# JuliaLinearAlgebra/AlgebraicMultigrid.jl

Measured on AMD Instinct MI355X. Metric: V-cycle unknowns/sec + fine-level SpMV GB/s (% HBM peak), 3-D Poisson 256^3, higher is better.
Workload: dtype f64

## Files before the change

### algebraicmultigrid.jl_amd/_libs.py

```python
import ctypes as C
import os

_HERE = os.path.dirname(os.path.abspath(__file__))
SETUP_SO = os.path.join(_HERE, "libamgsetup.so")
HIP_SO = os.path.join(_HERE, "libamghip.so")
HIP_F32_SO = os.path.join(_HERE, "libamghip_f32.so")

i32p = C.POINTER(C.c_int32)
f64p = C.POINTER(C.c_double)
i64 = C.c_int64
vp = C.c_void_p


class AMGError(RuntimeError):
    pass


class amgs_options(C.Structure):
    _fields_ = [("theta", C.c_double), ("max_levels", C.c_int32), ("max_coarse", C.c_int32),
                ("hermitian", C.c_int32), ("sa_omega", C.c_double), ("sa_improve_iters", C.c_int32),
                ("sa_B_is_vector", C.c_int32)]


class amgh_smoother_t(C.Structure):
# ... 144 lines not shown
    L.amgh_stream.restype = vp
    L.amgh_stream.argtypes = [vp]
    L.amgh_timer_begin.argtypes = [vp]
    L.amgh_timer_end.argtypes = [vp, C.POINTER(C.c_double)]
    L.amgh_bench_op.argtypes = [vp, C.c_int, C.c_int, C.c_int, C.c_int, C.POINTER(C.c_double)]
    L.amgh_debug_chain_timing.argtypes = [C.c_int, vp]
    L.amgh_debug_merged_sweep_host.argtypes = [i64, i64, vp, vp, vp, C.c_int, C.c_int, C.c_double, vp, vp]
    L.amgh_debug_bw_poll_giveups.argtypes = [vp, C.c_int]
    L.amgh_debug_bw_mode.argtypes = [vp, C.c_int]
    L.amgh_debug_bw_dict.argtypes = [vp, C.c_int]
    L.amgh_debug_bw_late.argtypes = [vp, C.c_int]
    L.amgh_debug_coded_ops.argtypes = [vp, C.c_int]
    L.amgh_debug_bw_sweep_host.argtypes = [i64, vp, vp, vp, C.c_int, C.c_int, C.c_double, vp, vp, vp]
    L.amgh_debug_bw_dict_sweep_host.argtypes = [i64, vp, vp, vp, C.c_int, C.c_int, vp, vp, vp]
    L.amgh_debug_set_tunable.argtypes = [C.c_char_p, C.c_int]
    L.amgh_debug_get_tunable.argtypes = [C.c_char_p, C.POINTER(C.c_int)]
    L.amgh_profile_enable.argtypes = [vp, C.c_int]
    L.amgh_profile_read.argtypes = [vp, vp, C.c_int]
    L.amgh_set_use_graph.argtypes = [vp, C.c_int]


def _bind_dist(L):
    i64p = C.POINTER(i64)
    L.amgh_dist_rccl_available.argtypes = []
    L.amgh_dist_unique_id.argtypes = [vp]
    L.amgh_dist_create_rccl.argtypes = [C.POINTER(vp), C.c_int, C.c_int, C.c_int, vp]
    L.amgh_local_group_create.argtypes = [C.POINTER(vp), C.c_int]
    L.amgh_local_group_destroy.argtypes = [vp]
    L.amgh_local_group_destroy.restype = None
    L.amgh_local_group_abort.argtypes = [vp]
# ... 97 lines not shown
```

### algebraicmultigrid.jl_amd/csrc/hip/amghip.hip

```cpp
#include "amghip_internal.hpp"
#include "gs_schedule.hpp"
#include "csr_ops.hpp"
#include "chebyshev.hpp"
#include "gmres_kernels.hpp"
#include "pcg_block_kernels.hpp"

namespace {

constexpr int64_t kGraphAutoRows = 65536;

struct Level {
  int64_t n = 0, nc = 0;
  amgh_csr A, S, P, R;
  bool has_S = false;
  amgh_smoother_t pre{}, post{};
  real *res = nullptr, *cx = nullptr, *cb = nullptr, *tmp = nullptr;
  real* cheb_d = nullptr;
  ChebSide cheb[2];
  const ChebSide& cheb_of(const amgh_smoother_t& s) const { return &s == &post ? cheb[1] : cheb[0]; }
  real* il = nullptr;
  amgh_csr* smat() { return has_S ? &S : &A; }
  amgh_csr Pp, Rp;
  bool lo_ok = false;
  real* lo_val = nullptr;
// ... 237 lines not shown
        RC_TRY(il_apply(bs, false, L->Rp.rowptr, L->Rp.col, L->Rp.val, nc, L->res, n, n, L->il, C ? cg->bp : L->cb, nc, h->stream, &L->Rp.cc));
      else
        RC_TRY(csr_apply(&L->Rp, M_SPMV, L->res, nullptr, C ? cg->bp : L->cb, h->stream, bs));
      if (C) cg->bp_cols = bs;
    }
    if (!C) RC_TRY(vec_fill(h, L->cx, nc * bs, 0.0));
    if (l == (int)h->levels.size() - 1) {
      ProfScope p(h, AMGH_T_COARSE, l + 1);
      for (int c = 0; c < bs; ++c) RC_TRY(coarse_solve(h, L->cx + c * nc, L->cb + c * nc));
    } else if (tail_here(h, l + 1, cyc) && (C != nullptr) == h->tail_lo) {
      ProfScope p(h, AMGH_T_COARSE, l + 1);
      RC_TRY(tail_apply(h, h->tail[cyc].M, nc, C ? cg->xp : L->cx, C ? cg->xstride : nc, C ? (const real*)cg->bp : (const real*)L->cb, nc, bs, false));
    } else {
      RC_TRY(cycle_next(h, l + 1, L->cx, L->cb, cyc, C != nullptr));
    }
    {
      ProfScope p(h, AMGH_T_PROLONG, l);
      if (L->il && il_block(bs) && !(L->p_stream && g_rhs_il == 1))
        RC_TRY(il_apply(bs, true, L->Pp.rowptr, L->Pp.col, L->Pp.val, n, C ? cg->xp : L->cx, nc, C ? cg->xstride : nc, L->il,
                        g->xp, xs, h->stream, &L->Pp.cc));
      else
        RC_TRY(raw_apply(M_ADD, L->Pp.rowptr, L->Pp.col, L->Pp.val, n, C ? cg->xp : L->cx, C ? cg->xstride : nc, nullptr, 0, g->xp,
                         xs, h->stream, bs, &L->Pp.cc));
    }
    {
      ProfScope p(h, AMGH_T_POSTSMOOTH, l);
      RC_TRY(smooth(h, L, L->post, xc, xo, b, bs, false, true, true,  lo_io));
    }
    return AMGH_OK;
  }
  {
    ProfScope p(h, AMGH_T_RESIDUAL, l);
    RC_TRY(csr_apply(&L->A, M_RESID, xc, b, L->res, h->stream, bs));
  }
  {
    ProfScope p(h, AMGH_T_RESTRICT, l);
    if (L->il && il_block(bs))
      RC_TRY(il_apply(bs, false, L->R.rowptr, L->R.col, L->R.val, nc, L->res, n, n, L->il, L->cb, nc, h->stream));
    else
      RC_TRY(csr_apply(&L->R, M_SPMV, L->res, nullptr, L->cb, h->stream, bs));
  }
  RC_TRY(vec_fill(h, L->cx, nc * bs, 0.0));
// ... 2075 lines not shown
  else if (!strcmp(name, "gs_bigslot")) *value = g_gs_bigslot;
  else if (!strcmp(name, "gs_super")) *value = g_gs_super;
  else if (!strcmp(name, "gs_block_pipe")) *value = g_gs_block_pipe;
  else return AMGH_EINVAL;
  return AMGH_OK;
}

int amgh_debug_set_perm_io(int on) {
  g_gs_flow_perm_io = on != 0;
  ++g_sched_epoch;
  return AMGH_OK;
}
int amgh_debug_get_perm_io(void) { return g_gs_flow_perm_io; }
int amgh_debug_perm_io_sweeps(int which) { return (which == 0 || which == 1) ? (int)(g_perm_io_sweeps[which] & 0x7fffffffu) : -1; }

int amgh_debug_chain_timing(int enable, unsigned long long* out8) {
  if (enable && !g_chain_tim) {
    HIP_TRY(hipMalloc((void**)&g_chain_tim, 8 * sizeof(unsigned long long)));
    HIP_TRY(hipMemset(g_chain_tim, 0, 8 * sizeof(unsigned long long)));
  }
  if (out8 && g_chain_tim) {
    HIP_TRY(hipDeviceSynchronize());
    HIP_TRY(hipMemcpy(out8, g_chain_tim, 8 * sizeof(unsigned long long), hipMemcpyDeviceToHost));
    HIP_TRY(hipMemset(g_chain_tim, 0, 8 * sizeof(unsigned long long)));
  }
  if (!enable && g_chain_tim) { hipFree(g_chain_tim); g_chain_tim = nullptr; }
  return AMGH_OK;
}

int amgh_profile_enable(amgh_t* h, int on) {
// ... 27 lines not shown
```

### algebraicmultigrid.jl_amd/csrc/hip/amghip_internal.hpp

```cpp
#pragma once
#include "amghip_kernels.hpp"
#include "gs_blocks.hpp"
#include "gs_flow.hpp"

#include <algorithm>
#include <chrono>
#include <cmath>
#include <cstdio>
#include <cstring>
#include <atomic>
#include <mutex>
#include <string>
#include <system_error>
#include <thread>
#include <utility>
#include <vector>

#include "../../../include/amghip.h"

using namespace amgh;

#define HIP_TRY(expr)                                   \
  do {                                                  \
    hipError_t e_ = (expr);                             \
// ... 286 lines not shown
    hipFree(rowmeta); hipFree(desc); hipFree(bp); hipFree(xp); hipFree(permx);
    d_lvl_ptr = rowptr = col = perm = dpos = nullptr; val = diag = bp = xp = nullptr; rowmeta = desc = nullptr; permx = nullptr;
  }
};

}

#include "dev_scan.hpp"

struct CodedCols {
  uint32_t* ccol = nullptr; real* vtab = nullptr; int n = 0;
  int64_t bytes = 0;
  void free_dev() { hipFree(ccol); hipFree(vtab); ccol = nullptr; vtab = nullptr; n = 0; bytes = 0; }
};

struct amgh_csr {
  CodedCols cc;
  bool cc_tried = false;
  bool xcd_map = false;
  int device = 0;
  int64_t nrows = 0, ncols = 0, nnz = 0;
  int32_t* rowptr = nullptr;
  int32_t* col = nullptr;
  real* val = nullptr;
  int32_t* dpos = nullptr;
  real* diag = nullptr;
  GsSchedule* gs = nullptr;
  int gs_nrhs_hint = 0;
  uint32_t pipe_epoch = 0; const void* pipe_rmbox = nullptr; int pipe_grid = 0;
  int64_t bytes = 0;
};

namespace {

int g_gs_block_pipe = 1;
int g_gs_super = 8;
int g_gs_coarse_lo = 1;
int g_gs_bigslot = 1;
int g_gs_merge = 16;
int g_jacobi_zero = 1;
int g_rhs_il = 1;
int g_gs_tiny = 1;
int g_gs_wave_quad = 1;
int g_gs_bw = 1;
int g_gs_bw_rows = 512;
int g_gs_bw_flow = 1;
int g_gs_bw_spin = 0;
int g_gs_bw_skip_pub = -1;
int g_gs_bw_nc = -1;
int g_gs_bw_nrhs = 1;
int g_gs_bw_chain = 1;
int g_stream_code = 1;
int g_trim_coded = 1;
int g_gs_bw_inorder = 0;
int g_gs_bw_dict = 1;
int g_gs_bw_relay = 3;
int g_gs_flow_xzero = 1;
int g_gs_flow_perm_io = 1;
unsigned int g_perm_io_sweeps[2] = {0, 0};
int g_gs_bw_two_min_rows = 200000;
int g_gs_sell = 1;
int g_gs_lean = -1;
int g_gs_ept = 0;
int g_gs_lpr = 0;
int g_gs_il = 1;
int g_pcg_fused = 1;
int g_tail_dense_rows = 6144;
int g_tail_dense = 1;
int g_gs_dense_blk = 4096;
int g_gs_dense_tri = 1;
int g_gs_block_inverse = 1;

std::atomic<unsigned long long> g_sched_epoch{0};

// ... 63 lines not shown
```

### algebraicmultigrid.jl_amd/csrc/hip/csr_ops.hpp

```cpp
#pragma once
#include <atomic>

namespace {


template <int MODE, class CFG = DefaultCfg, bool CODED = false>
int launch_stream(const StreamArgs& a0, hipStream_t st, int ncolv = 1) {
  const int nrows = a0.row_end - a0.row_begin;
  if (nrows <= 0) return AMGH_OK;
  StreamArgs a = a0;
  a.ncolv = ncolv;
  const int nb = (nrows + CFG::ROWS - 1) / CFG::ROWS;
  const int64_t grid = (CFG::XCD || ncolv > 1) ? (int64_t)((nb + kNumXcd - 1) / kNumXcd) * kNumXcd * ncolv : nb;
  hipLaunchKernelGGL((csr_stream_kernel<MODE, CFG, CODED>), dim3((unsigned)grid), dim3(CFG::THREADS), 0, st, a);
  HIP_TRY(hipGetLastError());
  return AMGH_OK;
}

constexpr int kGsBlockTarget = 256;
constexpr int kGsMinRows = 4;
constexpr int kGsNnzPerWg = 256;
template <int MODE>
int launch_gs_level(const StreamArgs& a, int rows, hipStream_t st, int ncolv = 1) {
  const int width = a.row_end - a.row_begin;
// ... 469 lines not shown
    void* fresh = nullptr;
    if (hipMalloc(&fresh, mb) != hipSuccess) { (void)hipGetLastError(); return AMGH_ENOMEM; }
    if (hipMemset(fresh, 0, mb) != hipSuccess) { (void)hipGetLastError(); (void)hipFree(fresh); return -1001; }
    (void)hipFree(g->bw.flow.mbox);
    g->bw.flow.mbox = fresh;
    const int64_t more = g->bw.flow.mail_stride * (int64_t)(ncolv - g->bw.flow.mcols);
    g->bw.flow.bytes += more; g->bw.rec_bytes += more; g->slot_bytes += more;
    grown += more;
    g->bw.flow.mcols = ncolv;
  }
  g->bytes += grown;
  op->bytes += grown;
  g->cols_alloc = ncolv;
  g->bp_cols = 0;
  return AMGH_OK;
}

int csr_gs_sweep(amgh_csr* op, bool backward, bool sor, real omega, real* x, const real* b, hipStream_t st,
                 bool first = true, bool last = true, int ncolv = 1, bool xzero = false, bool reuse_b = false,
                 bool x_resident = false, bool no_scatter = false, bool sym_pair = false) {
  RC_TRY(csr_ensure_gs(op));
  GsSchedule* g = op->gs;
  if (g->n <= 0) return AMGH_OK;
  if (sym_pair && (backward || !gs_wave_path(g, sor))) return AMGH_EINVAL;
  RC_TRY(gs_ensure_cols(op, ncolv, st));
  if (g->dti_f && g_gs_dense_tri && g_gs_block_inverse && !sor) {
    g->bp_cols = 0;
    const GsSchedule::Tri& t = backward ? g->dtri_b : g->dtri_f;
    const int B = g->dti_B, nb = (int)g->dti_off.size() - 1;
    for (int q = 0; q < nb; ++q) {
// ... 84 lines not shown
  if (first || !il) g->xil_cols = 0;
  bool il_s_ok = false;
  if (il && g->xil_cap < xs * ncolv) {
    HIP_TRY(hipStreamSynchronize(st));
    ++g_sched_epoch;
    hipFree(g->xil); g->xil = nullptr; g->xil_cap = 0;
    RC_TRY(dev_alloc(&g->xil, xs * ncolv));
    g->xil_cap = xs * ncolv;
    g->bytes += (int64_t)sizeof(real) * xs * ncolv; op->bytes += (int64_t)sizeof(real) * xs * ncolv;
    g->xil_cols = 0;
  }
  const bool perm_io = g_gs_flow_perm_io && ncolv == 1 && g->ncols == g->n && lay == g && !op->pipe_epoch && g_gs_bw_relay > 0 &&
                       g->bw.on && g->bw.flow.on && (g_gs_bw_flow || !g->bw.rec) &&
                       (int64_t)sizeof(real) * g->n < 0x7ffffff0ll;
  const bool fuse_b = perm_io && first && !(reuse_b && g->bp_cols == ncolv);
  const bool fuse_x = perm_io && last && !no_scatter && bw::relay_perm_x_ok<real>(g->bw.maxk, g->bw.flow.dict_on && (g_gs_bw_dict || !g->bw.flow.srec)) &&
                      ((g->bw.flow.dict_on && (g_gs_bw_dict || !g->bw.flow.srec)) ? g->bw.flow.dict_lds : g->bw.flow.lds_max) + bw::relay_perm_lds<real>(g->bw.flow.lds_max) <= 64 * 1024;
  if (first) {
    if (!(reuse_b && g->bp_cols == ncolv) && !fuse_b)
      hipLaunchKernelGGL(gather_perm_kernel, dim3(grid_for(g->n), ncolv), dim3(256), 0, st, b, g->perm, g->bp, (int)g->n,
                         (int64_t)g->n, (int64_t)g->n);
    g->bp_cols = ncolv;
    if (x_resident) {
    } else if (xzero) {
      const bool flow_zero = g_gs_flow_xzero && g->bw.on && g->bw.flow.on && (g_gs_bw_flow || !g->bw.rec) && g->ncols == g->n && lay == g;
      if (!flow_zero) {
        const int64_t cnt = xs * ncolv;
        hipLaunchKernelGGL(fill_kernel, dim3(grid_for(cnt)), dim3(256), 0, st, g->xp, cnt, 0.0);
        if (il) {
          const int64_t ci = g->ncols * ncolv;
// ... 73 lines not shown
      if (ncolv > g->bw.flow.mcols) return AMGH_ESTATE;
      const bool dict = g->bw.flow.dict_on && (g_gs_bw_dict || !g->bw.flow.srec);
      if (op->pipe_epoch) {
        if (ncolv != 1 || !g->bw.flow.xon) return AMGH_ESTATE;
        fa.aux = g->bw.flow.xaux; fa.fl_mb = g->bw.flow.xfl_mb; fa.fl_slot = g->bw.flow.xfl_slot; fa.xlist = g->bw.flow.xlist;
        fa.epoch = op->pipe_epoch; fa.rmbox = op->pipe_rmbox; fa.grid = op->pipe_grid;
        if (dict) { fa.crec = g->bw.flow.crec; fa.dict = g->bw.flow.dict; fa.dict_ent = g->bw.flow.dict_ent; }
        e = bw::sweep_relay<real>(fa, g->bw.maxk, dict ? g->bw.flow.dict_lds : g->bw.flow.lds_max, sor, backward, st, BW_RELAY_W);
      } else if (ncolv == 1 && g_gs_bw_relay > 0) {
        constexpr int kBwGrid = 0, kBwGridLong = 512;
        fa.grid = g->bw.maxk > 6 ? (dict ? 0 : kBwGridLong) : kBwGrid;
        fa.late = (g->bw.flow.late_ok && !g_gs_bw_inorder) ? 1 : 0;
        if (dict) { fa.crec = g->bw.flow.crec; fa.dict = g->bw.flow.dict; fa.dict_ent = g->bw.flow.dict_ent; }
        if (fuse_b) { fa.perm_b = g->perm; fa.b_nat = b; }
        if (fuse_x) { fa.perm_x = g->perm; fa.x_nat = x; }
        if (fuse_b || fuse_x) {
          e = bw::sweep_relay_io<real>(fa, g->bw.maxk, dict ? g->bw.flow.dict_lds : g->bw.flow.lds_max, g->bw.flow.lds_max, sor, backward, st);
          g_perm_io_sweeps[0] += fuse_b ? 1u : 0u; g_perm_io_sweeps[1] += fuse_x ? 1u : 0u;
        } else
        e = bw::sweep_relay<real>(fa, g->bw.maxk, dict ? g->bw.flow.dict_lds : g->bw.flow.lds_max, sor, backward, st, BW_RELAY_W);
      } else {
        if (dict) {
          fa.crec = g->bw.flow.crec; fa.dict = g->bw.flow.dict; fa.dict_ent = g->bw.flow.dict_ent;
          fa.dict_lds = (int32_t)(g->bw.flow.dict_lds - g->bw.flow.lds_max);
        }
        e = bw::sweep_flow<real>(fa, g->bw.maxk, g->bw.flow.lds_max, sor, backward, st, ncolv, g_gs_bw_nc >= 0 ? g_gs_bw_nc : (fa.crec ? 3 : 2));
      }
    } else {
      bw::Args<real> ba{g->bw.blocks, g->bw.rec, g->bw.ext_col, rhs, xp, ldb, xs, omega, 0, nullptr};
      if (g_gs_bw_chain && ncolv == 1 && g->bw.flags) {
        bw::ChainArgs<real> ca{ba, backward ? g->bw.sdep_ptr : g->bw.dep_ptr, backward ? g->bw.sdep : g->bw.dep, g->bw.flags, g->bw.head,
                               g->bw.nblocks, g->bw.err};
        e = bw::sweep_chain<real>(ca, g->bw.maxk, g->bw.lds_max, sor, backward, st);
      } else {
        e = bw::sweep<real>(ba, g->bw.maxk, g->bw.launch_ptr, g->bw.lds_max, sor, backward, ncolv, st);
      }
// ... 119 lines not shown
```

### algebraicmultigrid.jl_amd/csrc/hip/gs_flow.hpp

```cpp
#pragma once
#include "gs_blocks.hpp"

namespace amgh {
namespace bw {

constexpr int32_t kPubFwd = 1 << 30;
constexpr int32_t kPubBwd = (int32_t)(1u << 31);
constexpr int32_t kPubMask = (1 << 30) - 1;
#ifndef BW_FLOW_WAVES
#define BW_FLOW_WAVES 4
#endif
#ifndef BW_FLOW_DEPTH
#define BW_FLOW_DEPTH 4
#endif

struct FlowDesc {
  int32_t aux;
  int32_t npost;
  int32_t pad0, pad1;
};
constexpr int kStepRowBits = 11, kStepCntBits = 7, kStepNeedMax = (1 << 14) - 1;
inline uint32_t step_word(int r0, int nr, int need) { return (uint32_t)r0 | ((uint32_t)nr << kStepRowBits) | ((uint32_t)need << (kStepRowBits + kStepCntBits)); }

constexpr int32_t kRemoteCell = (int32_t)(1u << 31);
// ... 361 lines not shown
  unsigned int spin_limit;
  int32_t skip_pub;
  int64_t ldb = 0, ldx = 0, mail_stride = 0;
  int32_t lds_stride = 0;
  int32_t ncols = 1, ngroups = 1;
  int32_t xzero = 0;
  uint32_t epoch = 0;
  const unsigned char* crec = nullptr; const unsigned char* dict = nullptr; const int32_t* dict_ent = nullptr;
  int32_t dict_lds = 0;
  const int32_t* xlist = nullptr;
  const void* rmbox = nullptr;
  int32_t late = 0;
  int32_t grid = 0;
  const int32_t* perm_b = nullptr; const R* b_nat = nullptr;
  const int32_t* perm_x = nullptr; R* x_nat = nullptr;
};

template <typename R> struct Mail;
template <> struct Mail<double> {
  static constexpr int kBytes = 16;
  typedef u32x4 cell;
  static __device__ __forceinline__ cell load(__amdgpu_buffer_rsrc_t rs, unsigned off) { return __builtin_amdgcn_raw_buffer_load_b128(rs, off, 0, 16); }
  static __device__ __forceinline__ cell load_sys(__amdgpu_buffer_rsrc_t rs, unsigned off) { return __builtin_amdgcn_raw_buffer_load_b128(rs, off, 0, 17); }
  static __device__ __forceinline__ void store(__amdgpu_buffer_rsrc_t rs, unsigned off, double v, unsigned epoch) {
    const unsigned long long u = (unsigned long long)__double_as_longlong(v);
    cell c; c.x = (unsigned)u; c.y = epoch; c.z = (unsigned)(u >> 32); c.w = epoch;
    __builtin_amdgcn_raw_buffer_store_b128(c, rs, off, 0, 16);
  }
  static __device__ __forceinline__ bool valid(const cell& c, unsigned epoch) { return c.y == epoch && c.w == epoch; }
  static __device__ __forceinline__ double value(const cell& c) { return __longlong_as_double((long long)(((unsigned long long)c.z << 32) | c.x)); }
// ... 533 lines not shown
```

### algebraicmultigrid.jl_amd/csrc/hip/gs_relay.hpp

```cpp
#pragma once
#include "gs_flow.hpp"

namespace amgh {
namespace bw {

#ifndef BW_RELAY_W
#define BW_RELAY_W 3
#endif

#ifndef BW_RELAY_SPIN
#define BW_RELAY_SPIN 48u
#endif
#ifndef BW_RELAY_DEPTH_SHORT
#define BW_RELAY_DEPTH_SHORT 3
#endif
#ifndef BW_RELAY_DEPTH_LONG
#define BW_RELAY_DEPTH_LONG 2
#endif
template <int MAXK> struct RelayDepth { static constexpr int value = MAXK <= 12 ? BW_RELAY_DEPTH_SHORT : BW_RELAY_DEPTH_LONG; };
#ifndef BW_RELAY_FETCH_SLEEP
#define BW_RELAY_FETCH_SLEEP 4
#endif
#ifndef BW_RELAY_FETCH_PD
#define BW_RELAY_FETCH_PD 1
#endif
#ifndef BW_RELAY_FETCH_GAP
#define BW_RELAY_FETCH_GAP 6
#endif
#ifndef BW_RELAY_DICT_DEPTH
#define BW_RELAY_DICT_DEPTH 3
#endif
template <int MAXK> struct RelayDepthD { static constexpr int value = BW_RELAY_DICT_DEPTH; };
template <int MAXK> struct RelayWaves { static constexpr int value = MAXK <= 6 ? 4 : MAXK <= 18 ? 2 : 1; };
template <int MAXK> struct RelayWavesD { static constexpr int value = MAXK <= 6 ? 5 : MAXK <= 18 ? 3 : 2; };

template <typename T> __device__ __forceinline__ T lds_get(unsigned addr) { return *(const __attribute__((address_space(3))) T*)(unsigned long long)addr; }
template <typename T> __device__ __forceinline__ void lds_put(unsigned addr, T v) { *(__attribute__((address_space(3))) T*)(unsigned long long)addr = v; }
__device__ __forceinline__ unsigned lds_addr(const void* p) { return (unsigned)(unsigned long long)(const __attribute__((address_space(3))) unsigned char*)p; }

template <typename R, bool SOR, bool BWD, int MAXK, int W, bool DICT, bool LATE, bool PB, bool PX>
__device__ __forceinline__ void relay_block(const FlowArgs<R>& a, unsigned char* lds_all, const int wv, const int lane, const unsigned int ut,
                                            const unsigned int epoch, const long long t_start) {
  typedef typename std::conditional<DICT, FlowOpsD<R, MAXK>, FlowOps<R, MAXK>>::type O;
  typedef Mail<R> M;
  constexpr int D = DICT ? RelayDepthD<MAXK>::value : RelayDepth<MAXK>::value;
  constexpr int RB = (int)sizeof(R);
  constexpr int NVC = FlowOps<R, MAXK>::NVC;
  const bool fetcher = wv == W;
  const int tk = (int)ut;
  const int ob = __builtin_amdgcn_readfirstlane(BWD ? a.nblocks - 1 - tk : tk);
  const Desc d = a.blocks[ob];
  const FlowDesc f = a.fd[ob];
  const int ns = d.nlev;
  const int nxb = (int)(((size_t)(d.nrows + d.next + 1) * sizeof(R) + 15) & ~(size_t)15);
  const unsigned spin_limit = a.spin_limit ? a.spin_limit : (1u << 22);
  unsigned char* lds = lds_all;
  R* xl = (R*)lds;
  unsigned int* ctl = (unsigned int*)(lds + nxb);
  R* x = a.x;
  if (fetcher) {
    constexpr int EU = 4;
    const R* xc = uniform_ptr(x);
    const int nfar = BWD ? d.npre + (d.next - d.npre - f.npost) : d.next - d.npre;
    if (a.xzero) {
      for (int e0 = 0; e0 < d.next; e0 += 64) { const int i = e0 + lane; if (i < d.next) xl[d.nrows + i] = (R)0; }
    } else
    for (int e0 = 0; e0 < nfar; e0 += 64 * EU) {
      int32_t ec[EU]; int es[EU];
#pragma unroll
      for (int k = 0; k < EU; ++k) {
        const int i = e0 + lane + 64 * k;
        es[k] = BWD ? (i < d.npre ? i : i + f.npost) : d.npre + i;
        ec[k] = a.ext_col[i < nfar ? d.ext0 + es[k] : 0];
      }
#pragma unroll
      for (int k = 0; k < EU; ++k) pin(ec[k]);
      R xe[EU];
#pragma unroll
      for (int k = 0; k < EU; ++k) xe[k] = xc[ec[k]];
#pragma unroll
      for (int k = 0; k < EU; ++k) pin(xe[k]);
#pragma unroll
      for (int k = 0; k < EU; ++k) { const int i = e0 + lane + 64 * k; if (i < nfar) xl[d.nrows + es[k]] = xe[k]; }
    }
    if (lane == 0) { xl[d.nrows + d.next] = (R)0; ctl[0] = 0u; ctl[1] = 0u; ctl[2] = 0u; ctl[3] = 0u; }
    fetcher_barrier();
#ifdef BW_RELAY_FETCH_PRIO
    __builtin_amdgcn_s_setprio(BW_RELAY_FETCH_PRIO);
#endif
    constexpr int U = 3;
    int nf = BWD ? f.npost : d.npre;
    int f0 = d.ext0 + (BWD ? d.npre : 0);
    if (a.xlist) {
      const int l0 = a.xlist[4 * (int64_t)ob], lf = a.xlist[4 * (int64_t)ob + 1], lb = a.xlist[4 * (int64_t)ob + 2];
// ... 155 lines not shown
#pragma unroll
      for (int c = 0; c < O::NCC - 1; ++c) asm_load<4>(o.cf[c], voff, rs_rec, s0 + (unsigned)(O::NVC + c) * sd);
      asm_load<O::CTAIL + 1>(o.ct, voff, rs_rec, s0 + (unsigned)(O::NVC + O::NCC - 1) * sd);
    }
    asm_load<RB / 4>(o.bb, (unsigned)tt * RB, rs_b, (unsigned)r0 * RB);
  };
  O ops[D];
  int perm_off = 0;
  {
    constexpr int XW = W >= 4 ? 2 : 4;
    if (a.xzero) {
      for (int p = wv * 64 + lane; p < d.nrows; p += 64 * W) xl[p] = (R)0;
    } else
    for (int p0 = wv * 64 * XW; p0 < d.nrows; p0 += 64 * XW * W) {
      R xv[XW];
#pragma unroll
      for (int k = 0; k < XW; ++k) { const int p = p0 + lane + 64 * k; xv[k] = x[d.row0 + (p < d.nrows ? p : 0)]; }
#pragma unroll
      for (int k = 0; k < XW; ++k) pin(xv[k]);
#pragma unroll
      for (int k = 0; k < XW; ++k) { const int p = p0 + lane + 64 * k; if (p < d.nrows) xl[p] = xv[k]; }
    }
    if constexpr (DICT) {
      const int32_t de = a.dict_ent[ob];
      const int nchunk = (((unsigned)de >> 24) + 1) * NVC;
      const u32x4* dg = (const u32x4*)(a.dict + (size_t)(de & 0xffffff) * 16);
      u32x4* dl = (u32x4*)(lds + nxb + 16);
      for (int i = wv * 64 + lane; i < nchunk; i += 64 * W) dl[i] = dg[i];
      perm_off = nchunk * 16;
    }
    if constexpr (PX) {
      perm_off += nxb + 16;
// ... 282 lines not shown
#endif
  if (a.tim && lane == 0) {
    long long* tt = a.tim + 4 * (int64_t)ob;
    if (wv == 0) {
      tt[0] = t_start; tt[1] = t_loaded;
      unsigned xcc = 0;
#ifdef BW_RELAY_STAMPS
      asm volatile("s_getreg_b32 %0, hwreg(HW_REG_XCC_ID)" : "=s"(xcc));
#endif
      tt[3] = (long long)(xcc & 15u);
    }
    if (wv == (ns - 1) % W) tt[2] = wall_clock64();
  }
}

template <typename R, bool SOR, bool BWD, int MAXK, int W, bool DICT = false, bool LATE = false, bool PB = false, bool PX = false>
__global__ __launch_bounds__(64 * (W + 1), DICT ? RelayWavesD<MAXK>::value : RelayWaves<MAXK>::value) void gs_bw_relay_kernel(FlowArgs<R> a) {
  extern __shared__ __attribute__((aligned(16))) unsigned char lds_all[];
  static_assert(W >= 2 && W <= 7, "walker waves per block");
#ifdef BW_RELAY_STAMPS
  static_assert(!PX, "the stamps of a measurement build lie where the slice of the permutation goes");
#endif
  const int wv = __builtin_amdgcn_readfirstlane((int)(threadIdx.x >> 6));
  const int lane = (int)(threadIdx.x & 63u);
  const unsigned int units = (unsigned int)a.nblocks;
  const bool persistent = gridDim.x < units;
  const unsigned int draws = units + (persistent ? gridDim.x : 0u);
  unsigned long long* s_ticket = (unsigned long long*)lds_all;
  if (blockIdx.x < 2048u) for (unsigned i = 0; i < (blockIdx.x >> 5); ++i) __builtin_amdgcn_s_sleep(14);
  for (;;) {
    const long long t_start = a.tim ? wall_clock64() : 0;
    if (threadIdx.x == 0) *s_ticket = atomicAdd(a.head, 1ull);
    __syncthreads();
    const unsigned long long tv = *s_ticket;
    const unsigned long long ticket = ((unsigned long long)(unsigned)__builtin_amdgcn_readfirstlane((int)(tv >> 32)) << 32) | (unsigned)__builtin_amdgcn_readfirstlane((int)tv);
    __syncthreads();
    const unsigned int ut = (unsigned int)ticket, sweeps = (unsigned int)(ticket >> 32);
    if (threadIdx.x == 0 && ut == draws - 1u)
      __hip_atomic_store(a.head, (unsigned long long)(sweeps + 2u >= 0x80000000u ? 0u : sweeps + 1u) << 32, __ATOMIC_RELAXED, __HIP_MEMORY_SCOPE_AGENT);
    if (ut >= units) return;
    const unsigned int epoch = a.epoch ? a.epoch : sweeps + 1u;
    relay_block<R, SOR, BWD, MAXK, W, DICT, LATE, PB, PX>(a, lds_all, wv, lane, ut, epoch, t_start);
    if (!persistent) return;
    __syncthreads();
  }
}
static_assert(RelayDepth<6>::value <= 4 && RelayDepth<12>::value <= 4 && RelayDepth<18>::value <= 4, "the first round of the relay's pipeline is written out for up to four sets");

inline size_t& relay_lds_pad() { static size_t pad = 0; return pad; }

template <typename R> inline size_t relay_perm_lds(size_t lds_x) {
  static_assert(sizeof(R) == 4 || sizeof(R) == 8, "4 bytes a row out of sizeof(R) bytes a row");
  return ((sizeof(R) == 8 ? (lds_x + 1) / 2 : lds_x) + 15) & ~(size_t)15;
}
template <typename R, bool SOR, bool BWD, int MAXK, int W, bool DICT = false, bool LATE = false, bool PB = false, bool PX = false>
inline hipError_t sweep_relay_launch(const FlowArgs<R>& a, size_t lds, hipStream_t st) {
  auto* fn = gs_bw_relay_kernel<R, SOR, BWD, MAXK, W, DICT, LATE, PB, PX>;
  if (relay_lds_pad()) {
    lds += relay_lds_pad();
    static hipError_t once = hipFuncSetAttribute((const void*)fn, hipFuncAttributeMaxDynamicSharedMemorySize, 160 * 1024);
    if (once != hipSuccess) return once;
    hipLaunchKernelGGL(fn, dim3((unsigned)(a.grid > 0 && a.grid < a.nblocks ? a.grid : a.nblocks)), dim3(64 * (W + 1)), lds, st, a);
    return hipGetLastError();
  }
#ifdef BW_RELAY_STAMPS
  lds += 128 * 24 + (DICT ? kDictLdsMax : 0);
#endif
  if (lds > 64 * 1024) return hipErrorInvalidValue;
  hipLaunchKernelGGL(fn, dim3((unsigned)(a.grid > 0 && a.grid < a.nblocks ? a.grid : a.nblocks)), dim3(64 * (W + 1)), lds, st, a);
  return hipGetLastError();
}
template <typename R, int MAXK, int W, bool DICT = false>
// ... 92 lines not shown
  if (px) return sweep_relay_io_k<R, MAXK, false, true>(a, lds, lds_x, sor, backward, st);
  return hipErrorInvalidValue;
}
template <typename R>
inline hipError_t sweep_relay_io(const FlowArgs<R>& a, int maxk, size_t lds_max, size_t lds_x, bool sor, bool backward, hipStream_t st) {
  switch (maxk) {
    case 6: return sweep_relay_io_m<R, 6>(a, lds_max, lds_x, sor, backward, st);
    case 12: return sweep_relay_io_m<R, 12>(a, lds_max, lds_x, sor, backward, st);
#if BW_PLAN_MAXK >= 18
    case 18: return sweep_relay_io_m<R, 18>(a, lds_max, lds_x, sor, backward, st);
#endif
  }
  return hipErrorInvalidValue;
}

}
}
```

### include/amghip.h

```cpp
#ifndef AMGHIP_H
#define AMGHIP_H

#include <stdint.h>

#ifdef __cplusplus
extern "C" {
#endif

#ifndef AMGH_REAL
#define AMGH_REAL double
#endif
typedef AMGH_REAL amgh_real;

typedef struct amgh_handle amgh_t;
typedef struct amgh_csr amgh_csr_t;

#define AMGH_OK 0
#define AMGH_EINVAL (-2)
#define AMGH_ESTATE (-3)
#define AMGH_ENOMEM (-4)
#define AMGH_EUNSUPPORTED (-5)

enum { AMGH_SMOOTH_NONE = 0, AMGH_SMOOTH_GS = 1, AMGH_SMOOTH_JACOBI = 2, AMGH_SMOOTH_SOR = 3, AMGH_SMOOTH_CHEBYSHEV = 4 };
enum { AMGH_SWEEP_FORWARD = 0, AMGH_SWEEP_BACKWARD = 1, AMGH_SWEEP_SYMMETRIC = 2 };
// ... 217 lines not shown
int amgh_debug_bw_dict_sweep_host(int64_t nrows, const int32_t* rowptr, const int32_t* col, const amgh_real* val, int target_rows,
                                  int backward, amgh_real* x, const amgh_real* b, int64_t* stats5);

int amgh_debug_bw_poll_giveups(const amgh_t* h, int l);

int amgh_debug_bw_mode(const amgh_t* h, int l);
int amgh_debug_bw_dict(const amgh_t* h, int l);
int amgh_debug_bw_late(const amgh_t* h, int l);
int amgh_debug_coded_ops(const amgh_t* h, int l);

int amgh_debug_set_tunable(const char* name, int value);
int amgh_debug_get_tunable(const char* name, int* value);
int amgh_debug_set_perm_io(int on);
int amgh_debug_get_perm_io(void);
int amgh_debug_perm_io_sweeps(int which);

int amgh_set_use_graph(amgh_t* h, int on);

#ifdef __cplusplus
}
#endif
#endif
```

Baseline: 1.211 billion.

## Fold prolongation correction into first post-smoothing Gauss-Seidel relay sweep

Instead of running a separate prolongation kernel (x += P*e) before post-smoothing, the first relay GS sweep now computes P*e per row as it loads x, reading P's rowptr, cols and values (or coded columns with a value table staged in LDS). This removes one kernel launch and one full read-modify-write pass over x per level. The cost is more loads inside the latency-sensitive sweep, extra LDS for the value table, changed launch bounds, and many eligibility conditions that fall back to the old path.

Measured after the change: 1.209 billion. No clear change (-0.1%).

```diff
diff --git a/algebraicmultigrid.jl_amd/_libs.py b/algebraicmultigrid.jl_amd/_libs.py
--- a/algebraicmultigrid.jl_amd/_libs.py
+++ b/algebraicmultigrid.jl_amd/_libs.py
@@ -182,6 +182,9 @@
     L.amgh_debug_bw_sweep_host.argtypes = [i64, vp, vp, vp, C.c_int, C.c_int, C.c_double, vp, vp, vp]
     L.amgh_debug_bw_dict_sweep_host.argtypes = [i64, vp, vp, vp, C.c_int, C.c_int, vp, vp, vp]
     L.amgh_debug_set_tunable.argtypes = [C.c_char_p, C.c_int]
+    L.amgh_debug_set_prolong_fold.argtypes = [C.c_int]
+    L.amgh_debug_get_prolong_fold.argtypes = []
+    L.amgh_debug_prolong_fold_sweeps.argtypes = []
     L.amgh_debug_get_tunable.argtypes = [C.c_char_p, C.POINTER(C.c_int)]
     L.amgh_profile_enable.argtypes = [vp, C.c_int]
     L.amgh_profile_read.argtypes = [vp, vp, C.c_int]
diff --git a/algebraicmultigrid.jl_amd/csrc/hip/amghip.hip b/algebraicmultigrid.jl_amd/csrc/hip/amghip.hip
--- a/algebraicmultigrid.jl_amd/csrc/hip/amghip.hip
+++ b/algebraicmultigrid.jl_amd/csrc/hip/amghip.hip
@@ -275,7 +275,11 @@
     } else {
       RC_TRY(cycle_next(h, l + 1, L->cx, L->cb, cyc, C != nullptr));
     }
-    {
+    ProlongFold pf;
+    pf.rowptr = L->Pp.rowptr; pf.cc = &L->Pp.cc; pf.col = L->Pp.col; pf.val = L->Pp.val;
+    pf.e = C ? cg->xp : L->cx; pf.nnz = L->Pp.nnz; pf.nc = nc;
+    const bool fold = !h->tail_building && !(L->il && il_block(bs)) && gs_prolong_fold_ok(L->smat(), L->post, bs, pf,  lo_io);
+    if (!fold) {
       ProfScope p(h, AMGH_T_PROLONG, l);
       if (L->il && il_block(bs) && !(L->p_stream && g_rhs_il == 1))
         RC_TRY(il_apply(bs, true, L->Pp.rowptr, L->Pp.col, L->Pp.val, n, C ? cg->xp : L->cx, nc, C ? cg->xstride : nc, L->il,
@@ -286,7 +290,11 @@
     }
     {
       ProfScope p(h, AMGH_T_POSTSMOOTH, l);
-      RC_TRY(smooth(h, L, L->post, xc, xo, b, bs, false, true, true,  lo_io));
+      amgh_csr* M = L->smat();
+      M->pfold = fold ? &pf : nullptr;
+      const int rc = smooth(h, L, L->post, xc, xo, b, bs, false, true, true,  lo_io);
+      M->pfold = nullptr;
+      RC_TRY(rc);
     }
     return AMGH_OK;
   }
@@ -2392,6 +2400,14 @@
 int amgh_debug_get_perm_io(void) { return g_gs_flow_perm_io; }
 int amgh_debug_perm_io_sweeps(int which) { return (which == 0 || which == 1) ? (int)(g_perm_io_sweeps[which] & 0x7fffffffu) : -1; }
 
+int amgh_debug_set_prolong_fold(int on) {
+  g_prolong_fold = on != 0;
+  ++g_sched_epoch;
+  return AMGH_OK;
+}
+int amgh_debug_get_prolong_fold(void) { return g_prolong_fold; }
+int amgh_debug_prolong_fold_sweeps(void) { return (int)(g_prolong_fold_sweeps & 0x7fffffffu); }
+
 int amgh_debug_chain_timing(int enable, unsigned long long* out8) {
   if (enable && !g_chain_tim) {
     HIP_TRY(hipMalloc((void**)&g_chain_tim, 8 * sizeof(unsigned long long)));
diff --git a/algebraicmultigrid.jl_amd/csrc/hip/amghip_internal.hpp b/algebraicmultigrid.jl_amd/csrc/hip/amghip_internal.hpp
--- a/algebraicmultigrid.jl_amd/csrc/hip/amghip_internal.hpp
+++ b/algebraicmultigrid.jl_amd/csrc/hip/amghip_internal.hpp
@@ -324,6 +324,11 @@
   void free_dev() { hipFree(ccol); hipFree(vtab); ccol = nullptr; vtab = nullptr; n = 0; bytes = 0; }
 };
 
+struct ProlongFold {
+  const int32_t* rowptr = nullptr; const CodedCols* cc = nullptr; const int32_t* col = nullptr; const real* val = nullptr;
+  const real* e = nullptr; int64_t nnz = 0, nc = 0;
+};
+
 struct amgh_csr {
   CodedCols cc;
   bool cc_tried = false;
@@ -338,6 +343,7 @@
   GsSchedule* gs = nullptr;
   int gs_nrhs_hint = 0;
   uint32_t pipe_epoch = 0; const void* pipe_rmbox = nullptr; int pipe_grid = 0;
+  const ProlongFold* pfold = nullptr;
   int64_t bytes = 0;
 };
 
@@ -368,6 +374,8 @@
 int g_gs_flow_xzero = 1;
 int g_gs_flow_perm_io = 1;
 unsigned int g_perm_io_sweeps[2] = {0, 0};
+int g_prolong_fold = 1;
+unsigned int g_prolong_fold_sweeps = 0;
 int g_gs_bw_two_min_rows = 200000;
 int g_gs_sell = 1;
 int g_gs_lean = -1;
diff --git a/algebraicmultigrid.jl_amd/csrc/hip/csr_ops.hpp b/algebraicmultigrid.jl_amd/csrc/hip/csr_ops.hpp
--- a/algebraicmultigrid.jl_amd/csrc/hip/csr_ops.hpp
+++ b/algebraicmultigrid.jl_amd/csrc/hip/csr_ops.hpp
@@ -507,6 +507,28 @@
   g->cols_alloc = ncolv;
   g->bp_cols = 0;
   return AMGH_OK;
+}
+
+static_assert(bw::kProlongTabMax == kCodeMax, "the value table of a coded operator");
+inline bool gs_prolong_fold_ok(const amgh_csr* op, const amgh_smoother_t& s, int ncolv, const ProlongFold& pf, bool no_scatter) {
+  const GsSchedule* g = op->gs;
+  if (!g_prolong_fold || ncolv != 1 || !g || s.iter < 1 || (s.kind != AMGH_SMOOTH_GS && s.kind != AMGH_SMOOTH_SOR)) return false;
+  if (g->n <= 0 || g->ncols != g->n || op->pipe_epoch || g_gs_bw_relay <= 0 || !g->bw.on || !g->bw.flow.on || !(g_gs_bw_flow || !g->bw.rec)) return false;
+  if (g_gs_merge > 1 && (g->mf || g->mb)) return false;
+  if (g->dti_f || g->nblk > 0 || g->bp_cols != 1) return false;
+  const bool coded = pf.cc && pf.cc->ccol && (g_stream_code || !pf.col);
+  if (!pf.rowptr || !pf.e || (!coded && !(pf.col && pf.val))) return false;
+  if (pf.nnz * (int64_t)std::max<size_t>(4, sizeof(real)) >= 0x7ffffff0ll || (pf.nc + 1) * (int64_t)sizeof(real) >= 0x7ffffff0ll || (g->n + 2) * 4 >= 0x7ffffff0ll) return false;
+  const bool dict = g->bw.flow.dict_on && (g_gs_bw_dict || !g->bw.flow.srec);
+  const bool late = g->bw.flow.late_ok && !g_gs_bw_inorder;
+  if (!bw::relay_prolong_ok<real>(g->bw.maxk, dict, late)) return false;
+  size_t lds = (dict ? g->bw.flow.dict_lds : g->bw.flow.lds_max) + bw::relay_prolong_lds<real>(coded);
+  const bool only = s.iter == 1 && s.sweep != AMGH_SWEEP_SYMMETRIC;
+  if (only && !no_scatter && g_gs_flow_perm_io && (int64_t)sizeof(real) * g->n < 0x7ffffff0ll) {
+    if (!bw::relay_perm_x_ok<real>(g->bw.maxk, dict)) return false;
+    lds += bw::relay_perm_lds<real>(g->bw.flow.lds_max);
+  }
+  return lds <= 64 * 1024;
 }
 
 int csr_gs_sweep(amgh_csr* op, bool backward, bool sor, real omega, real* x, const real* b, hipStream_t st,
@@ -621,6 +643,7 @@
                        g->bw.on && g->bw.flow.on && (g_gs_bw_flow || !g->bw.rec) &&
                        (int64_t)sizeof(real) * g->n < 0x7ffffff0ll;
   const bool fuse_b = perm_io && first && !(reuse_b && g->bp_cols == ncolv);
+  const bool fuse_p = first && op->pfold != nullptr;
   const bool fuse_x = perm_io && last && !no_scatter && bw::relay_perm_x_ok<real>(g->bw.maxk, g->bw.flow.dict_on && (g_gs_bw_dict || !g->bw.flow.srec)) &&
                       ((g->bw.flow.dict_on && (g_gs_bw_dict || !g->bw.flow.srec)) ? g->bw.flow.dict_lds : g->bw.flow.lds_max) + bw::relay_perm_lds<real>(g->bw.flow.lds_max) <= 64 * 1024;
   if (first) {
@@ -724,12 +747,21 @@
         if (dict) { fa.crec = g->bw.flow.crec; fa.dict = g->bw.flow.dict; fa.dict_ent = g->bw.flow.dict_ent; }
         if (fuse_b) { fa.perm_b = g->perm; fa.b_nat = b; }
         if (fuse_x) { fa.perm_x = g->perm; fa.x_nat = x; }
-        if (fuse_b || fuse_x) {
+        if (fuse_p) {
+          const ProlongFold& pf = *op->pfold;
+          if (fuse_b || fa.xzero || lay != g) return AMGH_ESTATE;
+          fa.pp_rowptr = pf.rowptr; fa.pp_e = pf.e;
+          if (pf.cc && pf.cc->ccol && (g_stream_code || !pf.col)) { fa.pp_ccol = pf.cc->ccol; fa.pp_vtab = pf.cc->vtab; fa.pp_vtab_n = pf.cc->n; }
+          else { fa.pp_col = pf.col; fa.pp_val = pf.val; }
+          e = bw::sweep_relay_pp<real>(fa, g->bw.maxk, dict ? g->bw.flow.dict_lds : g->bw.flow.lds_max, g->bw.flow.lds_max, sor, backward, st);
+          ++g_prolong_fold_sweeps; g_perm_io_sweeps[1] += fuse_x ? 1u : 0u;
+        } else if (fuse_b || fuse_x) {
           e = bw::sweep_relay_io<real>(fa, g->bw.maxk, dict ? g->bw.flow.dict_lds : g->bw.flow.lds_max, g->bw.flow.lds_max, sor, backward, st);
           g_perm_io_sweeps[0] += fuse_b ? 1u : 0u; g_perm_io_sweeps[1] += fuse_x ? 1u : 0u;
         } else
         e = bw::sweep_relay<real>(fa, g->bw.maxk, dict ? g->bw.flow.dict_lds : g->bw.flow.lds_max, sor, backward, st, BW_RELAY_W);
       } else {
+        if (first && op->pfold) return AMGH_ESTATE;
         if (dict) {
           fa.crec = g->bw.flow.crec; fa.dict = g->bw.flow.dict; fa.dict_ent = g->bw.flow.dict_ent;
           fa.dict_lds = (int32_t)(g->bw.flow.dict_lds - g->bw.flow.lds_max);
diff --git a/algebraicmultigrid.jl_amd/csrc/hip/gs_flow.hpp b/algebraicmultigrid.jl_amd/csrc/hip/gs_flow.hpp
--- a/algebraicmultigrid.jl_amd/csrc/hip/gs_flow.hpp
+++ b/algebraicmultigrid.jl_amd/csrc/hip/gs_flow.hpp
@@ -399,6 +399,9 @@
   int32_t grid = 0;
   const int32_t* perm_b = nullptr; const R* b_nat = nullptr;
   const int32_t* perm_x = nullptr; R* x_nat = nullptr;
+  const int32_t* pp_rowptr = nullptr; const uint32_t* pp_ccol = nullptr; const R* pp_vtab = nullptr; int32_t pp_vtab_n = 0;
+  const int32_t* pp_col = nullptr; const R* pp_val = nullptr;
+  const R* pp_e = nullptr;
 };
 
 template <typename R> struct Mail;
diff --git a/algebraicmultigrid.jl_amd/csrc/hip/gs_relay.hpp b/algebraicmultigrid.jl_amd/csrc/hip/gs_relay.hpp
--- a/algebraicmultigrid.jl_amd/csrc/hip/gs_relay.hpp
+++ b/algebraicmultigrid.jl_amd/csrc/hip/gs_relay.hpp
@@ -34,11 +34,60 @@
 template <int MAXK> struct RelayWaves { static constexpr int value = MAXK <= 6 ? 4 : MAXK <= 18 ? 2 : 1; };
 template <int MAXK> struct RelayWavesD { static constexpr int value = MAXK <= 6 ? 5 : MAXK <= 18 ? 3 : 2; };
 
+template <typename R, int MAXK, bool DICT, bool LATE> struct RelayWavesP {
+  static constexpr int base = DICT ? RelayWavesD<MAXK>::value : RelayWaves<MAXK>::value;
+  static constexpr int want = MAXK <= 6 ? (DICT ? (sizeof(R) == 4 ? 7 : LATE ? 6 : 5) : (sizeof(R) == 4 ? 6 : 4)) : 0;
+  static constexpr int value = want > base ? want : base;
+};
 template <typename T> __device__ __forceinline__ T lds_get(unsigned addr) { return *(const __attribute__((address_space(3))) T*)(unsigned long long)addr; }
 template <typename T> __device__ __forceinline__ void lds_put(unsigned addr, T v) { *(__attribute__((address_space(3))) T*)(unsigned long long)addr = v; }
 __device__ __forceinline__ unsigned lds_addr(const void* p) { return (unsigned)(unsigned long long)(const __attribute__((address_space(3))) unsigned char*)p; }
 
-template <typename R, bool SOR, bool BWD, int MAXK, int W, bool DICT, bool LATE, bool PB, bool PX>
+constexpr int kProlongTabMax = 256;
+template <typename R> __device__ __forceinline__ R relay_buf_get(__amdgpu_buffer_rsrc_t rs, unsigned off) {
+  if constexpr (sizeof(R) == 8) {
+    const u32x2 t = __builtin_amdgcn_raw_buffer_load_b64(rs, off, 0, 0);
+    return __hiloint2double((int)t.y, (int)t.x);
+  } else return __uint_as_float(__builtin_amdgcn_raw_buffer_load_b32(rs, off, 0, 0));
+}
+template <typename R, int N, typename I>
+__device__ __forceinline__ void relay_prolong(const FlowArgs<R>& a, const unsigned vt, const I (&row)[N], R (&xv)[N]) {
+  static_assert(N % 2 == 0, "two rows at a time");
+  const bool coded = a.pp_ccol != nullptr;
+  const __amdgpu_buffer_rsrc_t rs_rp = __builtin_amdgcn_make_buffer_rsrc(uniform_ptr(const_cast<int32_t*>(a.pp_rowptr)), 0, 0x7ffffff0, 0x00020000);
+  const __amdgpu_buffer_rsrc_t rs_ent = __builtin_amdgcn_make_buffer_rsrc(uniform_ptr(coded ? (void*)const_cast<uint32_t*>(a.pp_ccol) : (void*)const_cast<int32_t*>(a.pp_col)), 0, 0x7ffffff0, 0x00020000);
+  const __amdgpu_buffer_rsrc_t rs_val = __builtin_amdgcn_make_buffer_rsrc(uniform_ptr(const_cast<R*>(coded ? a.pp_vtab : a.pp_val)), 0, 0x7ffffff0, 0x00020000);
+  const __amdgpu_buffer_rsrc_t rs_e = __builtin_amdgcn_make_buffer_rsrc(uniform_ptr(const_cast<R*>(a.pp_e)), 0, 0x7ffffff0, 0x00020000);
+  constexpr unsigned RB = (unsigned)sizeof(R);
+#pragma unroll
+  for (int h = 0; h < N; h += 2) {
+    int i0 = (int)__builtin_amdgcn_raw_buffer_load_b32(rs_rp, (unsigned)row[h] * 4u, 0, 0), e0 = (int)__builtin_amdgcn_raw_buffer_load_b32(rs_rp, (unsigned)row[h] * 4u + 4u, 0, 0);
+    int i1 = (int)__builtin_amdgcn_raw_buffer_load_b32(rs_rp, (unsigned)row[h + 1] * 4u, 0, 0), e1 = (int)__builtin_amdgcn_raw_buffer_load_b32(rs_rp, (unsigned)row[h + 1] * 4u + 4u, 0, 0);
+    R acc0 = (R)0, acc1 = (R)0;
+    unsigned w0 = __builtin_amdgcn_raw_buffer_load_b32(rs_ent, i0 < e0 ? (unsigned)i0 * 4u : 0u, 0, 0), w1 = __builtin_amdgcn_raw_buffer_load_b32(rs_ent, i1 < e1 ? (unsigned)i1 * 4u : 0u, 0, 0);
+    while (i0 < e0 || i1 < e1) {
+      const bool on0 = i0 < e0, on1 = i1 < e1;
+      const unsigned c0 = w0, c1 = w1;
+      R v0, v1;
+      if (!coded) { v0 = relay_buf_get<R>(rs_val, on0 ? (unsigned)i0 * RB : 0u); v1 = relay_buf_get<R>(rs_val, on1 ? (unsigned)i1 * RB : 0u); }
+      ++i0; ++i1;
+      w0 = __builtin_amdgcn_raw_buffer_load_b32(rs_ent, i0 < e0 ? (unsigned)i0 * 4u : 0u, 0, 0); w1 = __builtin_amdgcn_raw_buffer_load_b32(rs_ent, i1 < e1 ? (unsigned)i1 * 4u : 0u, 0, 0);
+      const R x0 = relay_buf_get<R>(rs_e, (coded ? (c0 & 0xffffffu) : c0) * RB), x1 = relay_buf_get<R>(rs_e, (coded ? (c1 & 0xffffffu) : c1) * RB);
+      if (coded) { v0 = lds_get<R>(vt + (c0 >> 24) * RB); v1 = lds_get<R>(vt + (c1 >> 24) * RB); }
+      if (on0) acc0 += v0 * x0;
+      if (on1) acc1 += v1 * x1;
+    }
+    xv[h] = xv[h] + acc0;
+    xv[h + 1] = xv[h + 1] + acc1;
+    pin(xv[h]); pin(xv[h + 1]);
+  }
+}
+template <typename R>
+__device__ __forceinline__ void relay_prolong_table(const FlowArgs<R>& a, const unsigned vt, const int lane) {
+  if (a.pp_ccol) for (int i = lane; i < a.pp_vtab_n; i += 64) lds_put<R>(vt + (unsigned)i * (unsigned)sizeof(R), a.pp_vtab[i]);
+}
+
+template <typename R, bool SOR, bool BWD, int MAXK, int W, bool DICT, bool LATE, bool PB, bool PX, bool PP>
 __device__ __forceinline__ void relay_block(const FlowArgs<R>& a, unsigned char* lds_all, const int wv, const int lane, const unsigned int ut,
                                             const unsigned int epoch, const long long t_start) {
   typedef typename std::conditional<DICT, FlowOpsD<R, MAXK>, FlowOps<R, MAXK>>::type O;
@@ -58,6 +107,15 @@
   R* xl = (R*)lds;
   unsigned int* ctl = (unsigned int*)(lds + nxb);
   R* x = a.x;
+  unsigned vt = 0u;
+  if constexpr (PP) {
+    static_assert(!PP || !PB, "a sweep that starts a smooth! call on a fresh b follows no prolongation");
+    unsigned o = (unsigned)nxb + 16u;
+    if constexpr (DICT) o += (((unsigned)a.dict_ent[ob] >> 24) + 1u) * (unsigned)(16 * NVC);
+    if constexpr (PX) o += ((unsigned)d.nrows * 4u + 15u) & ~15u;
+    vt = (unsigned)__builtin_amdgcn_readfirstlane((int)(lds_addr(lds) + o));
+    relay_prolong_table<R>(a, vt, lane);
+  }
   if (fetcher) {
     constexpr int EU = 4;
     const R* xc = uniform_ptr(x);
@@ -78,6 +136,7 @@
       R xe[EU];
 #pragma unroll
       for (int k = 0; k < EU; ++k) xe[k] = xc[ec[k]];
+      if constexpr (PP) relay_prolong<R, EU>(a, vt, ec, xe);
 #pragma unroll
       for (int k = 0; k < EU; ++k) pin(xe[k]);
 #pragma unroll
@@ -263,8 +322,15 @@
     } else
     for (int p0 = wv * 64 * XW; p0 < d.nrows; p0 += 64 * XW * W) {
       R xv[XW];
+      if constexpr (PP) {
+        int rw[XW];
+#pragma unroll
+        for (int k = 0; k < XW; ++k) { const int p = p0 + lane + 64 * k; rw[k] = d.row0 + (p < d.nrows ? p : 0); xv[k] = x[rw[k]]; }
+        relay_prolong<R, XW>(a, vt, rw, xv);
+      } else {
 #pragma unroll
       for (int k = 0; k < XW; ++k) { const int p = p0 + lane + 64 * k; xv[k] = x[d.row0 + (p < d.nrows ? p : 0)]; }
+      }
 #pragma unroll
       for (int k = 0; k < XW; ++k) pin(xv[k]);
 #pragma unroll
@@ -577,8 +643,8 @@
   }
 }
 
-template <typename R, bool SOR, bool BWD, int MAXK, int W, bool DICT = false, bool LATE = false, bool PB = false, bool PX = false>
-__global__ __launch_bounds__(64 * (W + 1), DICT ? RelayWavesD<MAXK>::value : RelayWaves<MAXK>::value) void gs_bw_relay_kernel(FlowArgs<R> a) {
+template <typename R, bool SOR, bool BWD, int MAXK, int W, bool DICT = false, bool LATE = false, bool PB = false, bool PX = false, bool PP = false>
+__global__ __launch_bounds__(64 * (W + 1), (PP ? RelayWavesP<R, MAXK, DICT, LATE>::value : DICT ? RelayWavesD<MAXK>::value : RelayWaves<MAXK>::value)) void gs_bw_relay_kernel(FlowArgs<R> a) {
   extern __shared__ __attribute__((aligned(16))) unsigned char lds_all[];
   static_assert(W >= 2 && W <= 7, "walker waves per block");
 #ifdef BW_RELAY_STAMPS
@@ -603,7 +669,7 @@
       __hip_atomic_store(a.head, (unsigned long long)(sweeps + 2u >= 0x80000000u ? 0u : sweeps + 1u) << 32, __ATOMIC_RELAXED, __HIP_MEMORY_SCOPE_AGENT);
     if (ut >= units) return;
     const unsigned int epoch = a.epoch ? a.epoch : sweeps + 1u;
-    relay_block<R, SOR, BWD, MAXK, W, DICT, LATE, PB, PX>(a, lds_all, wv, lane, ut, epoch, t_start);
+    relay_block<R, SOR, BWD, MAXK, W, DICT, LATE, PB, PX, PP>(a, lds_all, wv, lane, ut, epoch, t_start);
     if (!persistent) return;
     __syncthreads();
   }
@@ -616,9 +682,9 @@
   static_assert(sizeof(R) == 4 || sizeof(R) == 8, "4 bytes a row out of sizeof(R) bytes a row");
   return ((sizeof(R) == 8 ? (lds_x + 1) / 2 : lds_x) + 15) & ~(size_t)15;
 }
-template <typename R, bool SOR, bool BWD, int MAXK, int W, bool DICT = false, bool LATE = false, bool PB = false, bool PX = false>
+template <typename R, bool SOR, bool BWD, int MAXK, int W, bool DICT = false, bool LATE = false, bool PB = false, bool PX = false, bool PP = false>
 inline hipError_t sweep_relay_launch(const FlowArgs<R>& a, size_t lds, hipStream_t st) {
-  auto* fn = gs_bw_relay_kernel<R, SOR, BWD, MAXK, W, DICT, LATE, PB, PX>;
+  auto* fn = gs_bw_relay_kernel<R, SOR, BWD, MAXK, W, DICT, LATE, PB, PX, PP>;
   if (relay_lds_pad()) {
     lds += relay_lds_pad();
     static hipError_t once = hipFuncSetAttribute((const void*)fn, hipFuncAttributeMaxDynamicSharedMemorySize, 160 * 1024);
@@ -741,5 +807,46 @@
   return hipErrorInvalidValue;
 }
 
-}
-}
+template <typename R, int MAXK, bool DICT, bool LATE> struct RelayProlong {
+  static constexpr bool ok = !(sizeof(R) == 8 && MAXK <= 6 && DICT && !LATE) && !(sizeof(R) == 4 && MAXK > 6 && MAXK <= 12 && DICT && LATE);
+};
+template <typename R> inline bool relay_prolong_ok(int maxk, bool dict, bool late) {
+  return !(sizeof(R) == 8 && maxk <= 6 && dict && !late) && !(sizeof(R) == 4 && maxk > 6 && maxk <= 12 && dict && late);
+}
+template <typename R> inline size_t relay_prolong_lds(bool coded) { return coded ? (size_t)kProlongTabMax * sizeof(R) : 0; }
+template <typename R, int MAXK, bool PX>
+inline hipError_t sweep_relay_pp_k(const FlowArgs<R>& a0, size_t lds, size_t lds_x, bool sor, bool backward, hipStream_t st) {
+  constexpr int W = BW_RELAY_W;
+  if (PX) lds += relay_perm_lds<R>(lds_x);
+  lds += relay_prolong_lds<R>(a0.pp_ccol != nullptr);
+  FlowArgs<R> a = a0;
+  a.ncols = 1; a.ngroups = 1; a.lds_stride = 0;
+  auto go = [&](auto dict, auto late) -> hipError_t {
+    constexpr bool DC = decltype(dict)::value, LT = decltype(late)::value;
+    if constexpr ((PX && !RelayPermX<R, MAXK, DC>::ok) || !RelayProlong<R, MAXK, DC, LT>::ok) return hipErrorInvalidValue;
+    else {
+      if (sor) return backward ? sweep_relay_launch<R, true, true, MAXK, W, DC, LT, false, PX, true>(a, lds, st) : sweep_relay_launch<R, true, false, MAXK, W, DC, LT, false, PX, true>(a, lds, st);
+      return backward ? sweep_relay_launch<R, false, true, MAXK, W, DC, LT, false, PX, true>(a, lds, st) : sweep_relay_launch<R, false, false, MAXK, W, DC, LT, false, PX, true>(a, lds, st);
+    }
+  };
+  if (a.crec) return a.late ? go(std::true_type(), std::true_type()) : go(std::true_type(), std::false_type());
+  return a.late ? go(std::false_type(), std::true_type()) : go(std::false_type(), std::false_type());
+}
+template <typename R>
+inline hipError_t sweep_relay_pp(const FlowArgs<R>& a, int maxk, size_t lds_max, size_t lds_x, bool sor, bool backward, hipStream_t st) {
+  if (!a.pp_rowptr || !a.pp_e || a.perm_b || a.xzero) return hipErrorInvalidValue;
+  if (a.pp_ccol ? (!a.pp_vtab || a.pp_vtab_n < 1 || a.pp_vtab_n > kProlongTabMax) : (!a.pp_col || !a.pp_val)) return hipErrorInvalidValue;
+  if (a.perm_x && !a.x_nat) return hipErrorInvalidValue;
+  const bool px = a.perm_x != nullptr;
+  switch (maxk) {
+    case 6: return px ? sweep_relay_pp_k<R, 6, true>(a, lds_max, lds_x, sor, backward, st) : sweep_relay_pp_k<R, 6, false>(a, lds_max, lds_x, sor, backward, st);
+    case 12: return px ? sweep_relay_pp_k<R, 12, true>(a, lds_max, lds_x, sor, backward, st) : sweep_relay_pp_k<R, 12, false>(a, lds_max, lds_x, sor, backward, st);
+#if BW_PLAN_MAXK >= 18
+    case 18: return px ? sweep_relay_pp_k<R, 18, true>(a, lds_max, lds_x, sor, backward, st) : sweep_relay_pp_k<R, 18, false>(a, lds_max, lds_x, sor, backward, st);
+#endif
+  }
+  return hipErrorInvalidValue;
+}
+
+}
+}
diff --git a/include/amghip.h b/include/amghip.h
--- a/include/amghip.h
+++ b/include/amghip.h
@@ -255,6 +255,9 @@
 int amgh_debug_set_perm_io(int on);
 int amgh_debug_get_perm_io(void);
 int amgh_debug_perm_io_sweeps(int which);
+int amgh_debug_set_prolong_fold(int on);
+int amgh_debug_get_prolong_fold(void);
+int amgh_debug_prolong_fold_sweeps(void);
 
 int amgh_set_use_graph(amgh_t* h, int on);
 
```
